# VCISwang/STCD

Measured on AMD Instinct MI355X. Metric: image-pairs/sec (256x256 bf16 SiamUnet_diff train), higher is better.
Workload: dtype bf16; 1 GPU; SiamUnet_diff(3,2) 256x256 full training step (fwd + cross_entropy + bwd + AdamW), 16 pairs/GPU, synthetic LEVIR-CD-shaped pairs resident in HBM; global_batch=16, image=256, parallelism=dp1

## Files before the change

### stcd_amd/csrc/common.h

```cpp
#pragma once
#include <hip/hip_runtime.h>
#include <stdint.h>
#include <stdio.h>
#include <stdlib.h>
#include <string>
#include <string.h>

#include "../../include/stcd_hip.h"

namespace stcd {

typedef __bf16 bf16;

enum DType { F32 = STCD_DTYPE_F32, BF16 = STCD_DTYPE_BF16 };
inline size_t dsize(int dt) { return dt == BF16 ? 2 : 4; }

void set_error(const std::string& msg);

static inline int env_int(const char* name, int dflt) { const char* v = getenv(name); return v ? atoi(v) : dflt; }
static inline bool env_flag(const char* name, bool dflt) { const char* v = getenv(name); return v && v[0] == (dflt ? '0' : '1') ? !dflt : dflt; }

#define STCD_CHECK(cond, msg)                                              \
    do {                                                                   \
        if (!(cond)) {                                                     \
// ... 157 lines not shown
}
__device__ __forceinline__ void xf_fold8(const float* __restrict__ tab_sc, const float* __restrict__ tab_sh, const float4 m0, const float4 m1,
                                         float (&sc)[8], float (&sh)[8]) {
    const float mk[8] = {m0.x, m0.y, m0.z, m0.w, m1.x, m1.y, m1.z, m1.w};
#pragma unroll
    for (int j = 0; j < 8; ++j) { sc[j] = tab_sc[j] * mk[j]; sh[j] = tab_sh[j] * mk[j]; }
}


void launch_in_pack(int dt, const float* x1, const float* x2, void* X, int B, int cin, int H, int W, hipStream_t s, int dates = 2);
void launch_gout_pack(int dt, const float* g, void* G, int B, int L, int H, int W, hipStream_t s, long long* bias_acc = nullptr);
struct BiasJob { int64_t acc_off; int64_t out_off; int C, valid; float scale; int pad_; };
void launch_bias_finish(const BiasJob* jobs_dev, int njobs, const char* ws, float* grads, hipStream_t s);

void launch_conv_ref(int dt, const stcd_conv_geom& g, const void* in, const float* w, int kpad, int wld,
                     const float* bias, void* out, bool out_nchw_f32, hipStream_t s);
void launch_wgrad_ref(int dt, const stcd_conv_geom& g, const void* in, const void* dout, float* dw, int kpad, int wld,
                      hipStream_t s);
void launch_wgrad_ref_f64(int dt, const stcd_conv_geom& g, const void* in, const void* dout, double* dw, int kpad, int wld,
                          hipStream_t s);

struct ConvMfmaPlan {
    int CiB = 0, nchunks = 0, KS = 0, modeB = 0, NT = 0, NTtot = 0;
    int64_t wf_elems = 0;
    bool ok = false;
};
ConvMfmaPlan conv_mfma_plan(const stcd_conv_geom& g);
void launch_pack_frag(const stcd_conv_geom& g, const ConvMfmaPlan& p, const float* w, int kpad, int wld, void* dst,
                      hipStream_t s);
int launch_conv_mfma(const stcd_conv_geom& g, const ConvMfmaPlan& p, const void* in, const void* wf, const float* bias,
                     void* out, bool out_nchw_f32, hipStream_t s);
int launch_conv_mfma_x4(const stcd_conv_geom g[4], const ConvMfmaPlan p[4], const void* in, const void* const wf[4],
                        const float* bias, void* out, hipStream_t s);
struct ConvResPlan {
    int NT = 0, CW = 32, nslices = 0, P = 0, blocks = 0;
    int filt_bytes = 0, lds_bytes = 0;
    int single_halo = 0;
    bool ok = false;
};
ConvResPlan conv_res_plan(const stcd_conv_geom& g, const ConvMfmaPlan& p, int groups);
struct BwdSum {
    const void* Y = nullptr; int ldy = 0;
    const float* stat = nullptr;
    const float* mask = nullptr;
    long long* acc = nullptr;
    int groups = 1;
};
int launch_conv_res(const stcd_conv_geom& g, const ConvMfmaPlan& p, const ConvResPlan& rp, const void* in, const void* wf,
                    const float* bias, void* out, int groups, long long* stat_acc, int cpad, hipStream_t s, int stat_c0 = 0,
                    float s1_scale = BN_FS1, float s2_scale = BN_FS2, const XfSrc* xf = nullptr, const BwdSum* bs = nullptr);
bool conv_res_bwdsum_ok(const stcd_conv_geom& g, const ConvResPlan& rp);
struct ConvTilePlan {
    int NT = 0, nparts = 0, nbuf = 0, nslices = 0, P = 0, blocks = 0, ntiles = 0;
    int filt_bytes = 0, lds_bytes = 0;
    bool ok = false;
};
ConvTilePlan conv_tile_plan(const stcd_conv_geom& g, const ConvMfmaPlan& p, int groups);
int launch_conv_tile(const stcd_conv_geom& g, const ConvMfmaPlan& p, const ConvTilePlan& tp, const void* in, const void* wf,
                     const float* bias, void* out, int groups, long long* stat_acc, int cpad, hipStream_t s, int stat_c0 = 0,
                     float s1_scale = BN_FS1, float s2_scale = BN_FS2);
struct ConvGemmPlan {
    int W = 0;
    int tiles_m = 0, tiles_n = 0, blocks = 0, lds_bytes = 0;
    int pix_chunks = 0;
    bool ok = false;
};
ConvGemmPlan conv_gemm_plan(const stcd_conv_geom& g, const ConvMfmaPlan& p, int groups);
struct ConvEpi {
    int relu = 0;
    const void* gate = nullptr; int ldg = 0;
    const void* res = nullptr; int ldr = 0;
    float alpha = 1.f, beta = 1.f;
};
int launch_conv_gemm(const stcd_conv_geom& g, const ConvMfmaPlan& p, const ConvGemmPlan& gp, const void* in, const void* wf,
                   const float* bias, void* out, int groups, long long* stat_acc, int cpad, hipStream_t s, int stat_c0 = 0,
                   float s1_scale = BN_FS1, float s2_scale = BN_FS2, const ConvEpi* epi = nullptr);
struct ConvHaloPlan {
    int NH = 0;
    int nslices = 0, P = 0, blocks = 0, lds_bytes = 0;
    bool ok = false;
};
ConvHaloPlan conv_halo_plan(const stcd_conv_geom& g, const ConvMfmaPlan& p);
int launch_conv_halo(const stcd_conv_geom& g, const ConvMfmaPlan& p, const ConvHaloPlan& hp, const void* in, const void* wf,
                     const float* bias, void* out, hipStream_t s, const ConvEpi* epi = nullptr);

struct ConvDmaPlan {
    int tiles_m = 0, tiles_n = 0, blocks = 0, lds_bytes = 0;
    bool ok = false;
};
ConvDmaPlan conv_dma_plan(const stcd_conv_geom& g, const ConvMfmaPlan& p);
int launch_conv_dma(const stcd_conv_geom& g, const ConvMfmaPlan& p, const ConvDmaPlan& dp, const void* in, const void* wf,
                    const float* bias, void* out, hipStream_t s, const ConvEpi* epi = nullptr);

bool conv_small_ok(const stcd_conv_geom& g, const ConvMfmaPlan& p);
int conv_small_blocks(const stcd_conv_geom& g, int groups);
int launch_conv_small(const stcd_conv_geom& g, const void* in, const void* wf_modeB, const float* bias, void* out,
                      bool out_nchw_f32, int groups, long long* stat_acc, int cpad, hipStream_t s, const XfSrc* xf = nullptr,
                      const BwdSum* bs = nullptr);
bool conv_small_bwdsum_ok(const stcd_conv_geom& g);
struct WgradMfmaPlan {
    int WCI = 1, NTW = 1, gx = 1, gy = 1, gz = 1;
    int64_t slab_floats = 0;
    int wi_valid = 0;
    int gemm = 0;
    int dma = 0;
    bool ok = false;
// ... 317 lines not shown
```

### stcd_amd/csrc/engine.hip

```cpp
#include <algorithm>
#include <climits>
#include <cstdint>
#include <array>
#include <cstring>
#include <memory>
#include <vector>

#include "common.h"

namespace stcd {

static thread_local std::string g_err;
void set_error(const std::string& msg) { g_err = msg; }

enum ConvKind { K_CONV3 = 0, K_CONVT3_S1 = 1, K_UPCONV = 2, K_CONV1 = 3, K_CONVT2 = 4, K_CONV3_S2 = 5, K_CONV1_S2 = 6, K_STEM7 = 7 };

struct TRef { int64_t off = -1; int ld = 0; };
struct GRef { int64_t off = -1; int ld = 0; int64_t goff = 0; };

static inline int round8(int c) { return (c + 7) & ~7; }

struct ConvW {
    std::string name;
    int kind = 0, cin = 0, cout = 0;
// ... 445 lines not shown
        if (e.convs[i].name == name) return (int)i;
    return -1;
}
static int bn_index(const stcd_engine& e, const std::string& name) {
    for (size_t i = 0; i < e.bns.size(); ++i)
        if (e.bns[i].name == name) return (int)i;
    return -1;
}

static stcd_conv_geom geom3(int N, int H, int W, int K, int ldi, int co, int ldo) {
    stcd_conv_geom g;
    memset(&g, 0, sizeof(g));
    g.n = N; g.hi = H; g.wi = W; g.ci = K; g.ldi = ldi;
    g.hm = H; g.wm = W; g.in_stride = 1;
    g.ho = H; g.wo = W; g.out_stride = 1; g.oy0 = 0; g.ox0 = 0;
    g.co = co; g.ldo = ldo;
    g.ntaps = 9;
    for (int t = 0; t < 9; ++t) { g.dy[t] = (int8_t)(t / 3 - 1); g.dx[t] = (int8_t)(t % 3 - 1); }
    return g;
}

static stcd_conv_geom geom_up_phase(const UpConv& U, int py, int px, int ldi, int ldo, int* tap0) {
    stcd_conv_geom g;
    memset(&g, 0, sizeof(g));
    g.n = U.N; g.hi = U.h; g.wi = U.w; g.ci = U.C; g.ldi = ldi;
    g.hm = U.h; g.wm = U.w; g.in_stride = 1;
    g.ho = U.Ho; g.wo = U.Wo; g.out_stride = 2; g.oy0 = py; g.ox0 = px;
    g.co = U.C; g.ldo = ldo;
    int t = 0;
    for (int dy = 0; dy <= py; ++dy)
        for (int dx = 0; dx <= px; ++dx) { g.dy[t] = (int8_t)dy; g.dx[t] = (int8_t)dx; ++t; }
    g.ntaps = t;
    static const int start[4] = {0, 1, 3, 5};
    *tap0 = start[py * 2 + px];
    return g;
}

static void conv_work(const stcd_engine& e, const stcd_conv_geom& g, int kreal, int nreal, double* flops, double* bytes);

static void pick_gemm_or_res(const stcd_engine& e, ConvOp& op, const stcd_conv_geom& g, int groups) {
    op.gemm = ConvGemmPlan();
    op.tile = ConvTilePlan();
    if (!e.use_gemm || op.small) return;
    if (op.res.ok && !(e.cf && op.res.NT == 1)) return;
    op.gemm = conv_gemm_plan(g, op.plan, groups);
    if (op.gemm.ok) op.res = ConvResPlan();
    static const bool halo_on = env_flag("STCD_HALO_KERNEL", false);
    op.halo = ConvHaloPlan();
    op.dma = ConvDmaPlan();
    if (op.gemm.ok && (int64_t)g.n * g.hm * g.wm >= 256 * 192) op.dma = conv_dma_plan(g, op.plan);
    if (halo_on && op.gemm.ok && (int64_t)g.n * ((g.hm + 15) / 16) * ((g.wm + 15) / 16) >= 512) op.halo = conv_halo_plan(g, op.plan);
}

constexpr int TILE_MAX_TILES = 512;
static void pick_tile(const stcd_engine& e, ConvOp& op, const stcd_conv_geom& g, int groups) {
    op.tile = ConvTilePlan();
    if (!e.use_tile || !op.res.ok || op.gemm.ok || op.small) return;
    const ConvTilePlan tp = conv_tile_plan(g, op.plan, groups);
    if (tp.ok && tp.ntiles <= TILE_MAX_TILES) op.tile = tp;
}

static WgradMfmaPlan pick_wgrad_plan(const stcd_engine& e, const stcd_conv_geom& g, int kpad, int wld) {
    if (e.use_gemm && e.use_wgroup && 2.0 * g.n * g.hm * g.wm * (double)g.ci * g.co >= 0.8e9) {
        WgradMfmaPlan p = wgrad_gemm_plan(g, kpad, wld);
        if (p.ok) return p;
    }
    if (e.use_wgroup && (g.ntaps == 9 || (e.cf && g.ntaps == 4)) && (int64_t)g.n * g.hm * g.wm >= 65536) {
        WgradMfmaPlan p = wgrad_dma_plan(g, kpad, wld);
        if (p.ok) return p;
    }
    return wgrad_mfma_plan(g, kpad, wld, is_snunet(e.arch) || (e.cf && g.ntaps == 9));
}

static bool same_group(const WgradGroup& G, const WgradOp& op) {
    const bool t9 = !op.plan.dma && op.g.ntaps == 9;
    return G.gemm == op.plan.gemm && G.dma == op.plan.dma && G.WCI == op.plan.WCI && G.NTW == op.plan.NTW && G.t9 == t9 && G.xf == (op.xf_C > 0);
}

static bool cf_side_on() { static const bool on = env_flag("STCD_CF_SIDE", true); return on; }

static void build_pack_jobs(stcd_engine& e, Bump& ws) {
    for (int st = 0; st < 2; ++st) { e.rjobs[st].clear(); e.rjobs_total[st] = 0; }
    for (int st = 0; st < 2; ++st) e.wgroups[st].clear();
    if (e.dt == BF16 && e.use_mfma) {
        if (e.use_wgroup) {
            for (WgradOp* op : e.wgrad_ops) {
                if (!op->plan.ok) continue;
                const bool t9 = !op->plan.dma && op->g.ntaps == 9;
                std::vector<WgradGroup>& gs = e.wgroups[op->stage];
                size_t gi = 0;
                while (gi < gs.size() && !same_group(gs[gi], *op)) ++gi;
                if (gi == gs.size()) { WgradGroup g; g.WCI = op->plan.WCI; g.NTW = op->plan.NTW; g.t9 = t9; g.gemm = op->plan.gemm; g.dma = op->plan.dma; g.xf = op->xf_C > 0; gs.push_back(g); }
                op->grouped = true;
            }
            for (int st = 0; st < 2; ++st)
                for (WgradGroup& G : e.wgroups[st]) {
                    if (G.gemm) { G.lds_bytes = 2 * 2 * G.gemm * (64 * 64 + 8 * 32); continue; }
                    if (G.dma) {
                        G.lds_bytes = 128 * 1024;
                        std::vector<WgradOp*> dops;
                        for (WgradOp* op : e.wgrad_ops)
                            if (op->grouped && op->stage == st && op->plan.dma) dops.push_back(op);
                        auto blocks_at = [&](int64_t kt) {
                            int64_t b = 0;
                            for (WgradOp* op : dops) {
                                const int64_t M = (int64_t)op->g.n * op->g.hi * op->g.wi;
                                b += ((M + kt * 64 - 1) / (kt * 64)) * op->plan.gy * op->plan.gz;
                            }
                            return b;
                        };
                        int64_t lo = 1, hi = 1;
                        const int dma_blocks = e.wg_side_on && cf_side_on() ? 192 : 256;
// ... 488 lines not shown
    hipStream_t s;
    template <typename P = void> P* at(int64_t off) const { return (P*)(ws + off); }
};

struct ProfScope {
    Prof& p; hipStream_t s; bool on; hipEvent_t b;
    ProfScope(const Ctx& c, int klass, double flops, double bytes, const char* kernel = nullptr);
    ~ProfScope() { if (on) (void)hipEventRecord(b, s); }
};

ProfScope::ProfScope(const Ctx& c, int klass, double flops, double bytes, const char* kernel)
    : p(c.e.prof), s(c.s), on(c.e.prof.on), b(nullptr) {
    if (!on) return;
    static const char* DEF[PC_COUNT] = {"k_conv", "k_wgrad", "k_bn_reduce<T, 0>", "k_bn_act", "k_bn_reduce<T, 1>", "k_bn_bwd_apply",
                                        "k_pool_bwd|k_fuse|k_slice", "k_pack_jobs|k_reduce_dw"};
    ProfRec r;
    r.a = p.get(); r.b = p.get(); r.klass = klass; r.flops = flops; r.bytes = bytes;
    r.name_id = p.intern(kernel ? kernel : DEF[klass]);
    b = r.b;
    p.recs.push_back(r);
    (void)hipEventRecord(r.a, s);
}

static void conv_work(const stcd_engine& e, const stcd_conv_geom& g, int kreal, int nreal, double* flops, double* bytes) {
    double pos = (double)g.n * g.hm * g.wm;
    *flops = 2.0 * pos * g.ntaps * kreal * nreal;
    double in_px = g.in_stride == 1 ? pos : (double)g.n * (2.0 * g.hm) * (2.0 * g.wm);
    *bytes = (in_px * kreal + pos * nreal + (double)g.ntaps * kreal * nreal) * (double)dsize(e.dt);
}

static bool mfma_on(const stcd_engine& e) { return e.dt == BF16 && e.use_mfma; }

struct StatReq { long long* acc = nullptr; int groups = 1; int c0 = 0; int C = 0; float s1 = BN_FS1, s2 = BN_FS2; };
static void exec_conv(const Ctx& c, const ConvOp& op, const void* in, const float* bias, void* out, bool nchw,
                      const StatReq* sr = nullptr, int* stat_chunks = nullptr, const ConvEpi* epi = nullptr, int* epi_fused = nullptr,
                      const XfSrc* xf = nullptr, const BwdSum* bs = nullptr) {
    const int stat_groups = (sr && sr->acc) ? sr->groups : 0;
    long long* stat_acc = sr ? sr->acc : nullptr;
    const bool bn_form = sr && sr->c0 == 0 && sr->C == op.g.co && sr->s1 == BN_FS1 && sr->s2 == BN_FS2;
    const ConvW& cv = c.e.convs[op.conv];
    const PackSpec& ps = op.dgrad ? cv.dgrad : cv.fwd;
    double fl, by;
    conv_work(c.e, op.g, op.kreal, op.nreal, &fl, &by);
    char kname[64];
    const bool gemm_path = mfma_on(c.e) && op.gemm.ok && op.wf >= 0 && !nchw;
    const bool small_path = !gemm_path && mfma_on(c.e) && op.small && op.wf >= 0 && c.e.use_small;
    const bool res_path = !gemm_path && !small_path && mfma_on(c.e) && op.res.ok && op.wf >= 0 && !nchw;
    const bool mfma_path = !small_path && !res_path && mfma_on(c.e) && op.plan.ok && op.wf >= 0;
    const bool tile_path = res_path && op.tile.ok && !(xf && xf->on) && !bs;
    const bool dma_path = gemm_path && op.dma.ok && op.res_groups == 1 && !(stat_groups > 0 && stat_acc);
    if (dma_path) snprintf(kname, sizeof(kname), "k_conv_dma");
    else if (gemm_path && op.halo.ok && !(stat_groups > 0 && stat_acc)) snprintf(kname, sizeof(kname), "k_conv_halo");
    else if (gemm_path) snprintf(kname, sizeof(kname), "k_conv_gemm<%d>", op.gemm.W);
    else if (tile_path) snprintf(kname, sizeof(kname), "k_conv_tile<%d>", op.tile.NT);
    else if (res_path) snprintf(kname, sizeof(kname), "k_conv_res<%d, %d, %s>", op.res.NT, op.res.CW, op.res.single_halo ? "true" : "false");
    else if (small_path) snprintf(kname, sizeof(kname), "k_conv_small<1, %d>", (op.g.ntaps * op.g.ci + 31) / 32 <= 5 ? 5 : 9);
    else if (mfma_path) snprintf(kname, sizeof(kname), "k_conv_mfma<%d>", op.plan.NT);
    else snprintf(kname, sizeof(kname), "k_conv_ref");
    if (bs) {
        ProfScope ps2(c, PC_CONV, fl, by + (double)op.g.n * op.g.ho * op.g.wo * op.g.co * 2.0, small_path ? "k_conv_small<bwd>" : "k_conv_res<bwd>");
        const int rc = small_path ? launch_conv_small(op.g, in, c.at(op.wf), bias, out, nchw, bs->groups, nullptr, op.g.co, c.s, nullptr, bs)
                                  : launch_conv_res(op.g, op.plan, op.res, in, c.at(op.wf), bias, out, op.res_groups, nullptr, op.g.co, c.s, 0,
                                                    BN_BS, BN_BS, nullptr, bs);
        if (rc != 0) set_error("fused BatchNorm-backward sums: the data-gradient launch does not fit its BWD kernel");
        return;
    }
    ProfScope prof(c, PC_CONV, fl, by, kname);
    if (stat_chunks) *stat_chunks = 0;
    if (epi_fused) *epi_fused = 0;
    if (dma_path && launch_conv_dma(op.g, op.plan, op.dma, in, c.at(op.wf), bias, out, c.s, epi) == 0) {
        if (epi_fused && epi) *epi_fused = 1;
        return;
    }
    if (gemm_path && op.halo.ok && !(stat_groups > 0 && stat_acc)) {
        if (launch_conv_halo(op.g, op.plan, op.halo, in, c.at(op.wf), bias, out, c.s, epi) == 0) {
            if (epi_fused && epi) *epi_fused = 1;
            return;
        }
    }
    if (gemm_path) {
        const bool want = stat_groups > 0 && stat_groups == op.res_groups && stat_acc;
        long long* sp = want ? stat_acc : nullptr;
        if (launch_conv_gemm(op.g, op.plan, op.gemm, in, c.at(op.wf), bias, out, op.res_groups, sp, want ? sr->C : op.g.co, c.s,
                           want ? sr->c0 : 0, want ? sr->s1 : BN_FS1, want ? sr->s2 : BN_FS2, epi) == 0) {
            if (stat_chunks && want) *stat_chunks = 1;
            if (epi_fused && epi) *epi_fused = 1;
            return;
        }
    }
    const bool xf_on = xf && xf->on;
    if (mfma_on(c.e) && op.small && op.wf >= 0 && c.e.use_small) {
        const int groups = xf_on ? xf->groups : (stat_groups > 0 && bn_form) ? stat_groups : 1;
        long long* sp = (stat_groups > 0 && bn_form && stat_groups == groups) ? stat_acc : nullptr;
        if (launch_conv_small(op.g, in, c.at(op.wf), bias, out, nchw, groups, sp, op.g.co, c.s, xf) == 0) {
            if (stat_chunks && sp) *stat_chunks = 1;
            return;
        }
    }
    if (tile_path) {
        const bool want = stat_groups > 0 && stat_groups == op.res_groups && stat_acc;
        long long* sp = want ? stat_acc : nullptr;
        if (launch_conv_tile(op.g, op.plan, op.tile, in, c.at(op.wf), bias, out, op.res_groups, sp, want ? sr->C : op.g.co, c.s,
                             want ? sr->c0 : 0, want ? sr->s1 : BN_FS1, want ? sr->s2 : BN_FS2) == 0) {
            if (stat_chunks && want) *stat_chunks = 1;
            return;
        }
    }
// ... 2242 lines not shown
    STCD_HIP(hipGetLastError());
    return 0;
}

static int check_geom(const stcd_conv_geom* g) {
    STCD_CHECK(g != nullptr, "geometry is null");
    STCD_CHECK(g->ntaps >= 1 && g->ntaps <= 9, "ntaps must be in [1,9]");
    STCD_CHECK(g->ci >= 8 && g->ci % 8 == 0 && g->ldi >= g->ci && g->ldi % 8 == 0, "ci/ldi must be multiples of 8");
    STCD_CHECK(g->co >= 1 && g->ldo >= g->co, "bad co/ldo");
    STCD_CHECK(g->in_stride >= 1 && g->out_stride >= 1 && g->n >= 1 && g->hm >= 1 && g->wm >= 1, "bad sizes");
    STCD_CHECK((g->hm - 1) * g->out_stride + g->oy0 < g->ho && (g->wm - 1) * g->out_stride + g->ox0 < g->wo,
               "output positions exceed the output buffer");
    return 0;
}
static int op_dma_splits(const stcd_conv_geom& g, const WgradMfmaPlan& p) {
    const int64_t M = (int64_t)g.n * g.hi * g.wi;
    return (int)std::max<int64_t>(1, std::min<int64_t>(256 / std::max(1, p.gy * p.gz), M / 512));
}
int64_t stcd_op_scratch_bytes(const stcd_conv_geom* g) {
    if (!g) return 0;
    ConvMfmaPlan p = conv_mfma_plan(*g);
    WgradMfmaPlan w = wgrad_mfma_plan(*g, g->ci, g->co), ww = wgrad_mfma_plan(*g, g->ci, g->co, true);
    WgradMfmaPlan wg = wgrad_gemm_plan(*g, g->ci, g->co);
    WgradMfmaPlan wd = wgrad_dma_plan(*g, g->ci, g->co);
    if (wd.ok) wgrad_dma_set_split(wd, *g, op_dma_splits(*g, wd), g->ci, g->co);
    return std::max<int64_t>(p.wf_elems * 2, std::max(std::max(std::max(w.slab_floats, ww.slab_floats), wg.ok ? wg.slab_floats : 0), wd.ok ? wd.slab_floats : 0) * 4) + 1024;
}
int stcd_op_conv(int dtype, int impl, const stcd_conv_geom* g, const void* in, const float* w, const float* bias,
                 void* out, void* scratch, int64_t scratch_bytes, void* hip_stream) {
    if (check_geom(g)) return 1;
    STCD_CHECK(in && w && out, "null pointer argument");
    if (impl == 1 || impl == 2 || impl == 3 || impl == 6 || impl == 8) {
        STCD_CHECK(dtype == STCD_DTYPE_BF16, "the MFMA implementation is bf16 only");
        ConvMfmaPlan p = conv_mfma_plan(*g);
        STCD_CHECK(p.ok, "geometry not supported by the MFMA kernel");
        STCD_CHECK(scratch && scratch_bytes >= p.wf_elems * 2, "scratch too small for the fragment-order filter");
        launch_pack_frag(*g, p, w, g->ci, g->co, scratch, (hipStream_t)hip_stream);
        if (impl == 3) {
            const ConvHaloPlan hp = conv_halo_plan(*g, p);
            STCD_CHECK(hp.ok, "geometry not supported by the resident-halo kernel (3x3 stride 1, Ci % 64 == 0, Co % 128 == 0)");
            STCD_CHECK(launch_conv_halo(*g, p, hp, in, scratch, bias, out, (hipStream_t)hip_stream) == 0, "launch failed");
            STCD_HIP(hipGetLastError());
            return 0;
        }
        if (impl == 6) {
            const ConvDmaPlan dp = conv_dma_plan(*g, p);
            STCD_CHECK(dp.ok, "geometry not supported by the LDS-DMA kernel (Ci % 64 == 0, Co % 256 == 0, (Ci / 64) * taps even and >= 4)");
            STCD_CHECK(launch_conv_dma(*g, p, dp, in, scratch, bias, out, (hipStream_t)hip_stream) == 0, "launch failed");
            STCD_HIP(hipGetLastError());
            return 0;
        }
        if (impl == 8) {
            const ConvTilePlan tp = conv_tile_plan(*g, p, 1);
            STCD_CHECK(tp.ok, "geometry not supported by the LDS-DMA tile kernel (3x3 stride 1 over the full map, Ci % 64 == 0, Co % 16 == 0)");
            STCD_CHECK(launch_conv_tile(*g, p, tp, in, scratch, bias, out, 1, nullptr, g->co, (hipStream_t)hip_stream) == 0, "launch failed");
            STCD_HIP(hipGetLastError());
            return 0;
        }
        if (impl == 1 && conv_small_ok(*g, p)) {
            STCD_CHECK(launch_conv_small(*g, in, scratch, bias, out, false, 1, nullptr, g->co, (hipStream_t)hip_stream) == 0,
                       "small-channel kernel rejected the geometry");
            STCD_HIP(hipGetLastError());
            return 0;
        }
        if (impl == 1 && !env_flag("STCD_NO_RES_KERNEL", false)) {
            const ConvResPlan rp = conv_res_plan(*g, p, 1);
            if (rp.ok && launch_conv_res(*g, p, rp, in, scratch, bias, out, 1, nullptr, g->co, (hipStream_t)hip_stream) == 0) {
                STCD_HIP(hipGetLastError());
                return 0;
            }
        }
        if (impl == 1 && !env_flag("STCD_NO_GEMM_KERNEL", false)) {
            const ConvGemmPlan gp = conv_gemm_plan(*g, p, 1);
            if (gp.ok && launch_conv_gemm(*g, p, gp, in, scratch, bias, out, 1, nullptr, g->co, (hipStream_t)hip_stream) == 0) {
                STCD_HIP(hipGetLastError());
                return 0;
            }
        }
        STCD_CHECK(launch_conv_mfma(*g, p, in, scratch, bias, out, false, (hipStream_t)hip_stream) == 0, "LDS budget exceeded");
        STCD_HIP(hipGetLastError());
        return 0;
    }
    STCD_CHECK(impl == 0, "impl must be 0 (reference FMA), 1 (MFMA, auto-selected kernel), 2 (generic MFMA kernel), 3 (resident-halo kernel), 6 (LDS-DMA kernel) or 8 (LDS-DMA tile kernel)");
    launch_conv_ref(dtype, *g, in, w, g->ci, g->co, bias, out, false, (hipStream_t)hip_stream);
    STCD_HIP(hipGetLastError());
    return 0;
}
int stcd_op_wgrad(int dtype, int impl, const stcd_conv_geom* g, const void* in, const void* dout, float* dw, void* scratch,
                  int64_t scratch_bytes, void* hip_stream) {
    if (check_geom(g)) return 1;
    STCD_CHECK(in && dout && dw, "null pointer argument");
    if (impl == 1 || impl == 4 || impl == 5) {
        STCD_CHECK(dtype == STCD_DTYPE_BF16, "the MFMA implementation is bf16 only");
        WgradMfmaPlan p = wgrad_mfma_plan(*g, g->ci, g->co, impl >= 4, impl == 5 ? 1 : 0);
        STCD_CHECK(p.ok, "geometry not supported by the MFMA kernel");
        STCD_CHECK(scratch && scratch_bytes >= p.slab_floats * 4, "scratch too small for the partial slabs");
        STCD_CHECK(launch_wgrad_mfma(*g, p, in, dout, (float*)scratch, g->ci, g->co, (hipStream_t)hip_stream) == 0, "LDS budget exceeded");
        launch_reduce_dw((const float*)scratch, p.gx, *g, g->ci, g->co, g->ci, g->co, nullptr, dw, (hipStream_t)hip_stream);
        STCD_HIP(hipGetLastError());
        return 0;
    }
    if (impl == 7) {
        STCD_CHECK(dtype == STCD_DTYPE_BF16, "the MFMA implementation is bf16 only");
        WgradMfmaPlan p = wgrad_dma_plan(*g, g->ci, g->co);
        STCD_CHECK(p.ok, "geometry not supported by the LDS-DMA weight-gradient kernel (stride 1, full map >= 64 wide, Ci % 256 == 0, Co % 256 == 0)");
        wgrad_dma_set_split(p, *g, op_dma_splits(*g, p), g->ci, g->co);
        const int64_t table = (p.slab_floats * 4 + 255) & ~(int64_t)255;
// ... 32 lines not shown
```

### stcd_amd/csrc/kernels_conv_tile.hip

```cpp
#include <algorithm>

#include "common.h"

namespace stcd {

typedef __attribute__((ext_vector_type(8))) __bf16 bf16x8;
typedef __attribute__((ext_vector_type(4))) float f32x4;
typedef __attribute__((ext_vector_type(2))) unsigned u32x2;

struct ConvTileArgs {
    stcd_conv_geom g;
    const bf16* in;
    const bf16* wf;
    const float* bias;
    bf16* out;
    int NTtot;
    int nparts, nbuf;
    int nslices, P, groups;
    int tiles_x, tiles_y, ntiles;
    int filt_bytes;
    long long* stat_acc;
    int cpad, stat_c0;
    float s1_scale, s2_scale;
    unsigned in_bytes, wf_bytes, out_bytes;
    int8_t tix[3][3];
};

constexpr int TL_HW = 18;
constexpr int TL_NDMA = 41;
constexpr int TL_PART = TL_NDMA * 1024;
constexpr int TL_NI = 11;
#define TL_LDS(P_) ((__attribute__((address_space(3))) void*)(P_))
#define TL_WAIT(N_) asm volatile("s_waitcnt vmcnt(%0)" ::"n"(N_) : "memory")

template <int NT>
__global__ void __launch_bounds__(256, NT == 4 ? 1 : 2)
k_conv_tile(const ConvTileArgs a) {
    extern __shared__ __attribute__((aligned(16))) char smem[];
    const int tid = threadIdx.x, lane = tid & 63;
    const int wid = __builtin_amdgcn_readfirstlane(tid >> 6);
    const int q = lane >> 4, r = lane & 15;
    const int P = a.P;
    const int bl = blockIdx.x % P, rest = blockIdx.x / P, slice = rest % a.nslices, grp = rest / a.nslices;
    char* const filt = smem;
    char* const halo0 = smem + a.filt_bytes;
    const int nparts = a.nparts, nbuf = a.nbuf;

    const int64_t lead = ((int64_t)a.g.wi + 1) * a.g.ldi * 2;
    const __amdgpu_buffer_rsrc_t xrs = __builtin_amdgcn_make_buffer_rsrc(
        const_cast<char*>(reinterpret_cast<const char*>(a.in)) - lead, (short)0, (int)(a.in_bytes + (unsigned)lead), 0x00020000);
    const __amdgpu_buffer_rsrc_t wrs = __builtin_amdgcn_make_buffer_rsrc(
        const_cast<char*>(reinterpret_cast<const char*>(a.wf)), (short)0, (int)a.wf_bytes, 0x00020000);
    const __amdgpu_buffer_rsrc_t ors = __builtin_amdgcn_make_buffer_rsrc(
        reinterpret_cast<char*>(a.out), (short)0, (int)a.out_bytes, 0x00020000);

    float bv[NT][4];
#pragma unroll
    for (int t2 = 0; t2 < NT; ++t2) {
        const int cb = (slice * NT + t2) * 16 + 4 * q;
        float4 b4 = make_float4(0.f, 0.f, 0.f, 0.f);
        if (a.bias) b4 = *reinterpret_cast<const float4*>(a.bias + cb);
        bv[t2][0] = b4.x; bv[t2][1] = b4.y; bv[t2][2] = b4.z; bv[t2][3] = b4.w;
    }
    asm volatile("s_waitcnt vmcnt(0)" ::: "memory");

    {
        const int nfrag = nparts * 2 * 9 * NT;
        for (int f0 = wid; f0 < nfrag + wid; f0 += 4) {
            const int f = min(f0, nfrag - 1);
            const int ntl = f % NT, ft = f / NT, t = ft % 9, c32 = ft / 9;
            const int src = (((c32 >> 1) * 9 + t) * 2 + (c32 & 1)) * a.NTtot + slice * NT + ntl;
            __builtin_amdgcn_raw_ptr_buffer_load_lds(wrs, TL_LDS(filt + f * 1024), 16, lane * 16,
                                                     __builtin_amdgcn_readfirstlane(src * 1024), 0, 0);
        }
    }

    int pyx[TL_NI], poff[TL_NI];
#pragma unroll
    for (int i = 0; i < TL_NI; ++i) {
        const int pix = min(wid + 4 * i, TL_NDMA - 1) * 8 + (lane >> 3);
        const int hx = pix % TL_HW, hy = pix / TL_HW;
        const int ch = (lane & 7) ^ ((hx >> 1) & 7);
        pyx[i] = pix < TL_HW * TL_HW ? (((hy - 1) << 16) | ((hx - 1) & 0xffff)) : (0x4000 << 16);
        poff[i] = ((hy * a.g.wi + hx) * a.g.ldi + ch * 8) * 2;
    }

    const int tpg = a.ntiles / a.groups;
// ... 115 lines not shown
                    acc[m][t2] = f32x4{0.f, 0.f, 0.f, 0.f};
                    u32x2 pk;
                    pk[0] = pack_bf16x2(v[0], v[1]);
                    pk[1] = pack_bf16x2(v[2], v[3]);
                    __builtin_amdgcn_raw_buffer_store_b64(pk, ors, inside ? (int)(obyte + t2 * 32) : (int)0x80000000u, 0, 0);
                    if (want_stats && inside) {
#pragma unroll
                        for (int j = 0; j < 4; ++j) {
                            const float rv = round_as<bf16>(v[j]);
                            s1[t2][j] += rv;
                            s2[t2][j] += rv * rv;
                        }
                    }
                }
            }
            stored = true;
        }
        TL_ADV(cur);
        buf = buf + 1 == nbuf ? 0 : buf + 1;
    }
#undef TL_ADV
#undef TL_REQ

    if (a.stat_acc) {
        float* red = reinterpret_cast<float*>(smem);
        __syncthreads();
#pragma unroll
        for (int t2 = 0; t2 < NT; ++t2)
#pragma unroll
            for (int j = 0; j < 4; ++j) {
                float x = s1[t2][j], y = s2[t2][j];
#pragma unroll
                for (int o = 1; o < 16; o <<= 1) { x += __shfl_xor(x, o, 64); y += __shfl_xor(y, o, 64); }
                if (r == 0) {
                    red[(((wid * NT + t2) * 4 + q) * 4 + j) * 2] = x;
                    red[(((wid * NT + t2) * 4 + q) * 4 + j) * 2 + 1] = y;
                }
            }
        __syncthreads();
        for (int i = tid; i < NT * 16 * 2; i += 256) {
            const int which = i / (NT * 16), c = i - which * NT * 16;
            const int t2 = c >> 4, qq = (c >> 2) & 3, j = c & 3;
            float acc_ = 0.f;
#pragma unroll
            for (int w = 0; w < 4; ++w) acc_ += red[(((w * NT + t2) * 4 + qq) * 4 + j) * 2 + which];
            const int chn = slice * NT * 16 + c - a.stat_c0;
            if (chn >= 0 && chn < a.cpad) bn_acc_add(a.stat_acc, bl, a.groups, a.cpad, grp, which, chn, acc_, which ? a.s2_scale : a.s1_scale);
        }
    }
}

ConvTilePlan conv_tile_plan(const stcd_conv_geom& g, const ConvMfmaPlan& p, int groups) {
    ConvTilePlan tp;
    if (!p.ok || p.modeB || p.CiB != 64 || g.ntaps != 9 || g.in_stride != 1 || g.out_stride != 1 || g.oy0 != 0 || g.ox0 != 0) return tp;
    if (g.ci % 64 != 0 || g.co % 16 != 0 || g.ldi % 8 != 0 || g.ldo % 4 != 0 || g.hm > g.hi || g.wm > g.wi) return tp;
    if (g.hm > g.ho || g.wm > g.wo) return tp;
    if (g.hi >= 16384 || g.wi >= 16384) return tp;
    if (groups < 1 || g.n % groups != 0) return tp;
    if (((int64_t)g.n * g.hi + 2) * g.wi * g.ldi * 2 >= ((int64_t)1 << 31)) return tp;
    if ((int64_t)g.n * g.ho * g.wo * g.ldo * 2 >= ((int64_t)1 << 31)) return tp;
    if ((int64_t)p.wf_elems * 2 >= ((int64_t)1 << 31)) return tp;
    bool seen[9] = {false};
    for (int t = 0; t < 9; ++t) {
        if (g.dy[t] < -1 || g.dy[t] > 1 || g.dx[t] < -1 || g.dx[t] > 1) return tp;
        seen[(g.dy[t] + 1) * 3 + g.dx[t] + 1] = true;
    }
    for (int t = 0; t < 9; ++t) if (!seen[t]) return tp;
    const int nparts = g.ci / 64, nbuf = std::min(nparts, 2), ntr = g.co / 16, cap = 160 * 1024 - 1024;
    auto lds_of = [&](int nt) { return nparts * 2 * 9 * nt * 1024 + nbuf * TL_PART; };
    int NT = 0;
    for (int nt = 4; nt >= 1 && !NT; nt >>= 1)
        if (ntr % nt == 0 && lds_of(nt) <= cap) NT = nt;
    if (!NT) return tp;
    if (NT == 4 && 2 * lds_of(2) <= cap) NT = 2;
    const int64_t tiles_x = (g.wm + 15) / 16, tiles_y = (g.hm + 15) / 16, ntiles = (int64_t)g.n * tiles_x * tiles_y;
    if (ntiles >= ((int64_t)1 << 24)) return tp;
    while (NT > 1 && ntiles * (ntr / NT) < 256) NT >>= 1;
    tp.NT = NT; tp.nparts = nparts; tp.nbuf = nbuf; tp.nslices = ntr / NT;
    tp.filt_bytes = nparts * 2 * 9 * NT * 1024;
    tp.lds_bytes = lds_of(NT);
    tp.ntiles = (int)ntiles;
    const int64_t tpg = ntiles / groups;
    const int per_cu = std::max(1, std::min(2, cap / tp.lds_bytes));
    const int64_t slots = (int64_t)per_cu * 256;
    const int64_t P = std::max<int64_t>(1, slots / ((int64_t)groups * tp.nslices));
    tp.P = (int)std::min<int64_t>(P, tpg);
    tp.blocks = tp.P * tp.nslices * groups;
    tp.ok = true;
    return tp;
}

int launch_conv_tile(const stcd_conv_geom& g, const ConvMfmaPlan& p, const ConvTilePlan& tp, const void* in, const void* wf,
                     const float* bias, void* out, int groups, long long* stat_acc, int cpad, hipStream_t s, int stat_c0, float s1_scale,
                     float s2_scale) {
    if (!tp.ok || groups < 1 || tp.blocks != tp.P * tp.nslices * groups) return 1;
    ConvTileArgs a;
    a.g = g;
    a.in = (const bf16*)in; a.wf = (const bf16*)wf; a.bias = bias; a.out = (bf16*)out;
    a.NTtot = p.NTtot; a.nparts = tp.nparts; a.nbuf = tp.nbuf;
    a.nslices = tp.nslices; a.P = tp.P; a.groups = groups;
    a.tiles_x = (g.wm + 15) / 16; a.tiles_y = (g.hm + 15) / 16; a.ntiles = g.n * a.tiles_x * a.tiles_y;
    a.filt_bytes = tp.filt_bytes;
    a.stat_acc = stat_acc; a.cpad = cpad; a.stat_c0 = stat_c0; a.s1_scale = s1_scale; a.s2_scale = s2_scale;
    a.in_bytes = (unsigned)((int64_t)g.n * g.hi * g.wi * g.ldi * 2);
    a.wf_bytes = (unsigned)(p.wf_elems * 2);
    a.out_bytes = (unsigned)((int64_t)g.n * g.ho * g.wo * g.ldo * 2);
    for (int t = 0; t < 9; ++t) a.tix[g.dy[t] + 1][g.dx[t] + 1] = (int8_t)t;
#define LAUNCH_TILE(N_)                                                                                           \
    do {                                                                                                          \
        static bool attr_set = false;                                                                             \
        if (!attr_set) {                                                                                          \
            (void)hipFuncSetAttribute((const void*)k_conv_tile<N_>, hipFuncAttributeMaxDynamicSharedMemorySize, 160 * 1024); \
            attr_set = true;                                                                                      \
        }                                                                                                         \
        k_conv_tile<N_><<<(unsigned)tp.blocks, 256, (size_t)tp.lds_bytes, s>>>(a);                                \
    } while (0)
    switch (tp.NT) {
        case 1: LAUNCH_TILE(1); break;
        case 2: LAUNCH_TILE(2); break;
        default: LAUNCH_TILE(4); break;
    }
#undef LAUNCH_TILE
    return 0;
}

}
```

Before: 7915 image-pairs/sec.

## Extend LDS-DMA tile conv kernel to 32-channel input parts and raise tile cap

Adds a templated tile-conv body that handles 32-channel input parts (CiB==32) with its own swizzle, multi-buffer halo ring (up to four buffers), and vmcnt-based waiting, so more 3x3 convs can take the LDS-DMA tile path instead of the res kernel. It also raises the maximum tile count eligible for the tile path from 512 to 1024, gated by a check that the stats partition matches the res plan. The goal is better overlap of halo loads with MFMA work on small-channel layers. Risks include lower arithmetic intensity per part and changed BN stat accumulation ordering.

```diff
diff --git a/stcd_amd/csrc/common.h b/stcd_amd/csrc/common.h
--- a/stcd_amd/csrc/common.h
+++ b/stcd_amd/csrc/common.h
@@ -233,6 +233,7 @@
 bool conv_res_bwdsum_ok(const stcd_conv_geom& g, const ConvResPlan& rp);
 struct ConvTilePlan {
     int NT = 0, nparts = 0, nbuf = 0, nslices = 0, P = 0, blocks = 0, ntiles = 0;
+    int PC = 64;
     int filt_bytes = 0, lds_bytes = 0;
     bool ok = false;
 };
diff --git a/stcd_amd/csrc/engine.hip b/stcd_amd/csrc/engine.hip
--- a/stcd_amd/csrc/engine.hip
+++ b/stcd_amd/csrc/engine.hip
@@ -521,12 +521,19 @@
     if (halo_on && op.gemm.ok && (int64_t)g.n * ((g.hm + 15) / 16) * ((g.wm + 15) / 16) >= 512) op.halo = conv_halo_plan(g, op.plan);
 }
 
-constexpr int TILE_MAX_TILES = 512;
+struct TilePick { int PC, max_tiles; };
+static const TilePick TILE_PICKS[] = {
+    {64, 1024},
+    {32, 1024},
+};
 static void pick_tile(const stcd_engine& e, ConvOp& op, const stcd_conv_geom& g, int groups) {
     op.tile = ConvTilePlan();
     if (!e.use_tile || !op.res.ok || op.gemm.ok || op.small) return;
     const ConvTilePlan tp = conv_tile_plan(g, op.plan, groups);
-    if (tp.ok && tp.ntiles <= TILE_MAX_TILES) op.tile = tp;
+    if (!tp.ok) return;
+    const bool same_sums = op.dgrad || tp.P == op.res.P || (tp.PC == 64 && tp.ntiles <= 512);
+    for (const TilePick& r : TILE_PICKS)
+        if (tp.PC == r.PC && tp.ntiles <= r.max_tiles && same_sums) { op.tile = tp; return; }
 }
 
 static WgradMfmaPlan pick_wgrad_plan(const stcd_engine& e, const stcd_conv_geom& g, int kpad, int wld) {
@@ -1121,7 +1128,7 @@
     if (dma_path) snprintf(kname, sizeof(kname), "k_conv_dma");
     else if (gemm_path && op.halo.ok && !(stat_groups > 0 && stat_acc)) snprintf(kname, sizeof(kname), "k_conv_halo");
     else if (gemm_path) snprintf(kname, sizeof(kname), "k_conv_gemm<%d>", op.gemm.W);
-    else if (tile_path) snprintf(kname, sizeof(kname), "k_conv_tile<%d>", op.tile.NT);
+    else if (tile_path) snprintf(kname, sizeof(kname), op.tile.PC == 64 ? "k_conv_tile<%d>" : "k_conv_tile_parts<%d, 32>", op.tile.NT);
     else if (res_path) snprintf(kname, sizeof(kname), "k_conv_res<%d, %d, %s>", op.res.NT, op.res.CW, op.res.single_halo ? "true" : "false");
     else if (small_path) snprintf(kname, sizeof(kname), "k_conv_small<1, %d>", (op.g.ntaps * op.g.ci + 31) / 32 <= 5 ? 5 : 9);
     else if (mfma_path) snprintf(kname, sizeof(kname), "k_conv_mfma<%d>", op.plan.NT);
@@ -3470,7 +3477,7 @@
         }
         if (impl == 8) {
             const ConvTilePlan tp = conv_tile_plan(*g, p, 1);
-            STCD_CHECK(tp.ok, "geometry not supported by the LDS-DMA tile kernel (3x3 stride 1 over the full map, Ci % 64 == 0, Co % 16 == 0)");
+            STCD_CHECK(tp.ok, "geometry not supported by the LDS-DMA tile kernel (3x3 stride 1 over the full map, Ci % 32 == 0, Co % 16 == 0)");
             STCD_CHECK(launch_conv_tile(*g, p, tp, in, scratch, bias, out, 1, nullptr, g->co, (hipStream_t)hip_stream) == 0, "launch failed");
             STCD_HIP(hipGetLastError());
             return 0;
diff --git a/stcd_amd/csrc/kernels_conv_tile.hip b/stcd_amd/csrc/kernels_conv_tile.hip
--- a/stcd_amd/csrc/kernels_conv_tile.hip
+++ b/stcd_amd/csrc/kernels_conv_tile.hip
@@ -27,12 +27,309 @@
 };
 
 constexpr int TL_HW = 18;
+constexpr int TL_MAXBUF = 4;
+template <int PC> struct TilePart {
+    static constexpr int NCH = PC / 8;
+    static constexpr int PPI = 64 / NCH;
+    static constexpr int NDMA = (TL_HW * TL_HW + PPI - 1) / PPI;
+    static constexpr int BYTES = NDMA * 1024;
+    static constexpr int NI = (NDMA + 3) / 4;
+    static constexpr int KS = PC / 32;
+};
+#define TL_LDS(P_) ((__attribute__((address_space(3))) void*)(P_))
+#define TL_WAIT(N_) asm volatile("s_waitcnt vmcnt(%0)" ::"n"(N_) : "memory")
+
+constexpr int TL_SWZ[TL_HW] = {3, 0, 1, 2, 7, 7, 5, 2, 3, 4, 4, 5, 7, 7, 0, 1, 3, 0};
+constexpr uint64_t tl_swz_pack() {
+    uint64_t v = 0;
+    for (int c = 0; c < TL_HW; ++c) v |= (uint64_t)TL_SWZ[c] << (3 * c);
+    return v;
+}
+constexpr uint64_t TL_SWZ_BITS = tl_swz_pack();
+template <int PC> __host__ __device__ constexpr int tl_swz(int col) {
+    return PC == 64 ? (int)((TL_SWZ_BITS >> (3 * col)) & 7) : (col >> 1) & 3;
+}
+template <int PC> constexpr bool tl_swz_conflict_free() {
+    constexpr int NCH = TilePart<PC>::NCH;
+    constexpr int g0[16] = {0, 1, 2, 3, 12, 13, 14, 15, 20, 21, 22, 23, 24, 25, 26, 27};
+    for (int c = 0; c < TL_HW; ++c)
+        if (tl_swz<PC>(c) < 0 || tl_swz<PC>(c) >= NCH) return false;
+    for (int row = 0; row < TL_HW; ++row)
+        for (int ks = 0; ks < TilePart<PC>::KS; ++ks)
+            for (int dx = 0; dx < 3; ++dx)
+                for (int grp = 0; grp < 4; ++grp) {
+                    unsigned seen = 0;
+                    for (int l = 0; l < 32; ++l) {
+                        bool in0 = false;
+                        for (int i = 0; i < 16; ++i) in0 = in0 || g0[i] == l;
+                        if (in0 != ((grp & 1) == 0)) continue;
+                        const int lane = l + 32 * (grp >> 1), q = lane >> 4, r = lane & 15;
+                        const int byte = ((row * TL_HW + r + dx) * NCH + ((ks * 4 + q) ^ tl_swz<PC>(r + dx))) * 16;
+                        const unsigned bit = 1u << ((byte >> 4) & 15);
+                        if (seen & bit) return false;
+                        seen |= bit;
+                    }
+                    if (seen != 0xffffu) return false;
+                }
+    return true;
+}
+static_assert(tl_swz_conflict_free<64>(), "a shifted halo fragment read has an LDS bank conflict (128-B pixel rows)");
+static_assert(tl_swz_conflict_free<32>(), "a shifted halo fragment read has an LDS bank conflict (64-B pixel rows)");
+
+__device__ __forceinline__ void tl_wait_vm(int n) {
+    switch (n) {
+#define TL_W1(N_) case N_: TL_WAIT(N_); break;
+#define TL_W8(N_) TL_W1(N_) TL_W1(N_ + 1) TL_W1(N_ + 2) TL_W1(N_ + 3) TL_W1(N_ + 4) TL_W1(N_ + 5) TL_W1(N_ + 6) TL_W1(N_ + 7)
+        TL_W8(0) TL_W8(8) TL_W8(16) TL_W8(24) TL_W8(32) TL_W8(40) TL_W8(48) TL_W8(56)
+#undef TL_W8
+#undef TL_W1
+        default: TL_WAIT(0); break;
+    }
+}
+
+template <int NT, int PC>
+__device__ __forceinline__ void conv_tile_body(const ConvTileArgs& a) {
+    using TP = TilePart<PC>;
+    constexpr int TL_NDMA = TP::NDMA, TL_PART = TP::BYTES, TL_NI = TP::NI, TL_KS = TP::KS, TL_NCH = TP::NCH, TL_PPI = TP::PPI;
+    extern __shared__ __attribute__((aligned(16))) char smem[];
+    const int tid = threadIdx.x, lane = tid & 63;
+    const int wid = __builtin_amdgcn_readfirstlane(tid >> 6);
+    const int q = lane >> 4, r = lane & 15;
+    const int P = a.P;
+    const int bl = blockIdx.x % P, rest = blockIdx.x / P, slice = rest % a.nslices, grp = rest / a.nslices;
+    char* const filt = smem;
+    char* const halo0 = smem + a.filt_bytes;
+    const int nparts = a.nparts, nbuf = a.nbuf;
+
+    const int64_t lead = ((int64_t)a.g.wi + 1) * a.g.ldi * 2;
+    const __amdgpu_buffer_rsrc_t xrs = __builtin_amdgcn_make_buffer_rsrc(
+        const_cast<char*>(reinterpret_cast<const char*>(a.in)) - lead, (short)0, (int)(a.in_bytes + (unsigned)lead), 0x00020000);
+    const __amdgpu_buffer_rsrc_t wrs = __builtin_amdgcn_make_buffer_rsrc(
+        const_cast<char*>(reinterpret_cast<const char*>(a.wf)), (short)0, (int)a.wf_bytes, 0x00020000);
+    const __amdgpu_buffer_rsrc_t ors = __builtin_amdgcn_make_buffer_rsrc(
+        reinterpret_cast<char*>(a.out), (short)0, (int)a.out_bytes, 0x00020000);
+
+    float bv[NT][4];
+#pragma unroll
+    for (int t2 = 0; t2 < NT; ++t2) {
+        const int cb = (slice * NT + t2) * 16 + 4 * q;
+        float4 b4 = make_float4(0.f, 0.f, 0.f, 0.f);
+        if (a.bias) b4 = *reinterpret_cast<const float4*>(a.bias + cb);
+        bv[t2][0] = b4.x; bv[t2][1] = b4.y; bv[t2][2] = b4.z; bv[t2][3] = b4.w;
+    }
+    asm volatile("s_waitcnt vmcnt(0)" ::: "memory");
+#pragma unroll
+    for (int t2 = 0; t2 < NT; ++t2)
+#pragma unroll
+        for (int j = 0; j < 4; ++j) asm volatile("" : "+v"(bv[t2][j]));
+
+    constexpr int TL_PF = TL_KS * 9 * NT, TL_NF = (TL_PF + 3) / 4;
+#define TL_REQ_FILT(C_)                                                                                                \
+    do {                                                                                                               \
+        _Pragma("unroll") for (int i = 0; i < TL_NF; ++i) {                                                            \
+            const int f = (C_) * TL_PF + min(wid + 4 * i, TL_PF - 1);                                                  \
+            const int ntl = f % NT, ft = f / NT, t = ft % 9, c32 = ft / 9;                                             \
+            const int src = (((c32 / TL_KS) * 9 + t) * TL_KS + c32 % TL_KS) * a.NTtot + slice * NT + ntl;              \
+            __builtin_amdgcn_raw_ptr_buffer_load_lds(wrs, TL_LDS(filt + f * 1024), 16, lane * 16,                      \
+                                                     __builtin_amdgcn_readfirstlane(src * 1024), 0, 0);                \
+        }                                                                                                              \
+    } while (0)
+
+    int pyx[TL_NI], poff[TL_NI];
+#pragma unroll
+    for (int i = 0; i < TL_NI; ++i) {
+        const int pix = min(wid + 4 * i, TL_NDMA - 1) * TL_PPI + lane / TL_NCH;
+        const int hx = pix % TL_HW, hy = pix / TL_HW;
+        const int ch = (lane % TL_NCH) ^ tl_swz<PC>(hx);
+        pyx[i] = pix < TL_HW * TL_HW ? (((hy - 1) << 16) | ((hx - 1) & 0xffff)) : (0x4000 << 16);
+        poff[i] = ((hy * a.g.wi + hx) * a.g.ldi + ch * 8) * 2;
+    }
+
+    const int tpg = a.ntiles / a.groups;
+    const int tiles_img = a.tiles_x * a.tiles_y;
+    const int dn = P / tiles_img, drem = P - dn * tiles_img, dty = drem / a.tiles_x, dtx = drem - dty * a.tiles_x;
+    const int tile0 = grp * tpg + bl;
+    const int tile_end = (grp + 1) * tpg;
+    struct Pos { int tile, n, y, x, c; };
+#define TL_ADV(P_)                                                                                                     \
+    do {                                                                                                               \
+        if (++(P_).c == nparts) {                                                                                      \
+            (P_).c = 0; (P_).tile += P;                                                                                \
+            (P_).x += dtx; if ((P_).x >= a.tiles_x) { (P_).x -= a.tiles_x; ++(P_).y; }                                 \
+            (P_).y += dty; if ((P_).y >= a.tiles_y) { (P_).y -= a.tiles_y; ++(P_).n; }                                 \
+            (P_).n += dn;                                                                                              \
+        }                                                                                                              \
+    } while (0)
+#define TL_REQ(P_, BUF_)                                                                                               \
+    do {                                                                                                               \
+        const int gy0_ = (P_).y * 16, gx0_ = (P_).x * 16;                                                               \
+        const int soff_ = __builtin_amdgcn_readfirstlane(                                                              \
+            (int)(((((int64_t)(P_).n * a.g.hi + gy0_) * a.g.wi + gx0_) * a.g.ldi + (P_).c * PC) * 2));                 \
+        char* const dst_ = halo0 + (BUF_) * TL_PART;                                                                   \
+        _Pragma("unroll") for (int i = 0; i < TL_NI; ++i) {                                                            \
+            const int hy_ = pyx[i] >> 16, hx_ = (int)(short)(pyx[i] & 0xffff);                                         \
+            const bool ok_ = (unsigned)(gy0_ + hy_) < (unsigned)a.g.hi && (unsigned)(gx0_ + hx_) < (unsigned)a.g.wi;   \
+            __builtin_amdgcn_raw_ptr_buffer_load_lds(xrs, TL_LDS(dst_ + min(wid + 4 * i, TL_NDMA - 1) * 1024), 16,     \
+                                                     ok_ ? poff[i] : (int)0x80000000u, soff_, 0, 0);                   \
+        }                                                                                                              \
+    } while (0)
+
+    Pos cur{tile0, 0, 0, 0, 0};
+    cur.n = tile0 / tiles_img;
+    { const int trem = tile0 - cur.n * tiles_img; cur.y = trem / a.tiles_x; cur.x = trem - cur.y * a.tiles_x; }
+    Pos rq = cur;
+    int inflight = 0;
+    for (int k = 0; k < nbuf; ++k) {
+        if (k < nparts) TL_REQ_FILT(k);
+        if (rq.tile < tile_end) { TL_REQ(rq, k); TL_ADV(rq); ++inflight; }
+    }
+    for (int k = nbuf; k < nparts; ++k) TL_REQ_FILT(k);
+#undef TL_REQ_FILT
+
+    float s1[NT][4], s2[NT][4];
+#pragma unroll
+    for (int t2 = 0; t2 < NT; ++t2)
+#pragma unroll
+        for (int j = 0; j < 4; ++j) s1[t2][j] = s2[t2][j] = 0.f;
+    f32x4 acc[4][NT];
+#pragma unroll
+    for (int m = 0; m < 4; ++m)
+#pragma unroll
+        for (int t2 = 0; t2 < NT; ++t2) acc[m][t2] = f32x4{0.f, 0.f, 0.f, 0.f};
+
+    int aoff[TL_KS][3];
+#pragma unroll
+    for (int ks = 0; ks < TL_KS; ++ks)
+#pragma unroll
+        for (int dx = 0; dx < 3; ++dx)
+            aoff[ks][dx] = (((4 * wid) * TL_HW + r + dx) * TL_NCH + ((ks * 4 + q) ^ tl_swz<PC>(r + dx))) * 16;
+
+    const bool want_stats = a.stat_acc != nullptr;
+    int buf = 0, step = 0;
+    unsigned ended = 0;
+    const unsigned ring = (1u << nbuf) - 1;
+    while (cur.tile < tile_end) {
+        {
+            const int ny = inflight - 1;
+            const int nst = __builtin_popcount(ended & ring);
+            tl_wait_vm(ny * TL_NI + nst * 4 * NT + (step < nbuf ? max(nparts - 1 - step, 0) * TL_NF : 0));
+            --inflight;
+        }
+        __builtin_amdgcn_s_barrier();
+        const char* hb = halo0 + buf * TL_PART;
+        {
+            bf16x8 ab[2][6], wb[2][3][NT];
+            const char* const fb0 = filt + (cur.c * TL_KS) * (9 * NT * 1024) + lane * 16;
+#define TL_LOAD_STAGE(S_, B_)                                                                                         \
+            do {                                                                                                      \
+                constexpr int ks_ = (S_) / 3, dx_ = (S_) % 3;                                                         \
+                _Pragma("unroll") for (int hr = 0; hr < 6; ++hr)                                                      \
+                    ab[B_][hr] = *reinterpret_cast<const bf16x8*>(hb + aoff[ks_][dx_] + hr * (TL_HW * PC * 2));       \
+                _Pragma("unroll") for (int dy = 0; dy < 3; ++dy)                                                      \
+                    _Pragma("unroll") for (int t2 = 0; t2 < NT; ++t2)                                                 \
+                        wb[B_][dy][t2] = *reinterpret_cast<const bf16x8*>(fb0 + ks_ * (9 * NT * 1024) + a.tix[dy][dx_] * (NT * 1024) + t2 * 1024); \
+            } while (0)
+#define TL_MMA_STAGE(B_)                                                                                              \
+            do {                                                                                                      \
+                _Pragma("unroll") for (int dy = 0; dy < 3; ++dy)                                                      \
+                    _Pragma("unroll") for (int t2 = 0; t2 < NT; ++t2)                                                 \
+                        _Pragma("unroll") for (int m = 0; m < 4; ++m)                                                 \
+                            acc[m][t2] = __builtin_amdgcn_mfma_f32_16x16x32_bf16(wb[B_][dy][t2], ab[B_][m + dy], acc[m][t2], 0, 0, 0); \
+            } while (0)
+            TL_LOAD_STAGE(0, 0);
+            TL_LOAD_STAGE(1, 1); __builtin_amdgcn_sched_barrier(0);
+            TL_MMA_STAGE(0);
+            TL_LOAD_STAGE(2, 0); __builtin_amdgcn_sched_barrier(0);
+            TL_MMA_STAGE(1);
+            if constexpr (TL_KS == 2) {
+                TL_LOAD_STAGE(3, 1); __builtin_amdgcn_sched_barrier(0);
+                TL_MMA_STAGE(0);
+                TL_LOAD_STAGE(4, 0); __builtin_amdgcn_sched_barrier(0);
+                TL_MMA_STAGE(1);
+                TL_LOAD_STAGE(5, 1); __builtin_amdgcn_sched_barrier(0);
+                TL_MMA_STAGE(0);
+                TL_MMA_STAGE(1);
+            } else {
+                TL_MMA_STAGE(0);
+            }
+#undef TL_LOAD_STAGE
+#undef TL_MMA_STAGE
+        }
+        barrier_lds();
+        if (rq.tile < tile_end) { TL_REQ(rq, buf); TL_ADV(rq); ++inflight; }
+        if (cur.c == nparts - 1) {
+            const int mx = cur.x * 16 + r;
+#pragma unroll
+            for (int m = 0; m < 4; ++m) {
+                const int my = cur.y * 16 + wid * 4 + m;
+                const bool inside = my < a.g.hm && mx < a.g.wm;
+                const unsigned obyte = (unsigned)(((((int64_t)cur.n * a.g.ho + my) * a.g.wo + mx) * a.g.ldo + slice * NT * 16 + 4 * q) * 2);
+#pragma unroll
+                for (int t2 = 0; t2 < NT; ++t2) {
+                    float v[4];
+#pragma unroll
+                    for (int j = 0; j < 4; ++j) v[j] = acc[m][t2][j] + bv[t2][j];
+                    acc[m][t2] = f32x4{0.f, 0.f, 0.f, 0.f};
+                    u32x2 pk;
+                    pk[0] = pack_bf16x2(v[0], v[1]);
+                    pk[1] = pack_bf16x2(v[2], v[3]);
+                    __builtin_amdgcn_raw_buffer_store_b64(pk, ors, inside ? (int)(obyte + t2 * 32) : (int)0x80000000u, 0, 0);
+                    if (want_stats && inside) {
+#pragma unroll
+                        for (int j = 0; j < 4; ++j) {
+                            const float rv = round_as<bf16>(v[j]);
+                            s1[t2][j] += rv;
+                            s2[t2][j] += rv * rv;
+                        }
+                    }
+                }
+            }
+        }
+        ended = (ended << 1) | (cur.c == nparts - 1 ? 1u : 0u);
+        TL_ADV(cur);
+        buf = buf + 1 == nbuf ? 0 : buf + 1;
+        ++step;
+    }
+#undef TL_ADV
+#undef TL_REQ
+
+    if (a.stat_acc) {
+        float* red = reinterpret_cast<float*>(smem);
+        __syncthreads();
+#pragma unroll
+        for (int t2 = 0; t2 < NT; ++t2)
+#pragma unroll
+            for (int j = 0; j < 4; ++j) {
+                float x = s1[t2][j], y = s2[t2][j];
+#pragma unroll
+                for (int o = 1; o < 16; o <<= 1) { x += __shfl_xor(x, o, 64); y += __shfl_xor(y, o, 64); }
+                if (r == 0) {
+                    red[(((wid * NT + t2) * 4 + q) * 4 + j) * 2] = x;
+                    red[(((wid * NT + t2) * 4 + q) * 4 + j) * 2 + 1] = y;
+                }
+            }
+        __syncthreads();
+        for (int i = tid; i < NT * 16 * 2; i += 256) {
+            const int which = i / (NT * 16), c = i - which * NT * 16;
+            const int t2 = c >> 4, qq = (c >> 2) & 3, j = c & 3;
+            float acc_ = 0.f;
+#pragma unroll
+            for (int w = 0; w < 4; ++w) acc_ += red[(((w * NT + t2) * 4 + qq) * 4 + j) * 2 + which];
+            const int chn = slice * NT * 16 + c - a.stat_c0;
+            if (chn >= 0 && chn < a.cpad) bn_acc_add(a.stat_acc, bl, a.groups, a.cpad, grp, which, chn, acc_, which ? a.s2_scale : a.s1_scale);
+        }
+    }
+}
+
+template <int NT, int PC>
+__global__ void __launch_bounds__(256, 2)
+k_conv_tile_parts(const ConvTileArgs a) {
+    conv_tile_body<NT, PC>(a);
+}
+
 constexpr int TL_NDMA = 41;
 constexpr int TL_PART = TL_NDMA * 1024;
 constexpr int TL_NI = 11;
-#define TL_LDS(P_) ((__attribute__((address_space(3))) void*)(P_))
-#define TL_WAIT(N_) asm volatile("s_waitcnt vmcnt(%0)" ::"n"(N_) : "memory")
-
 template <int NT>
 __global__ void __launch_bounds__(256, NT == 4 ? 1 : 2)
 k_conv_tile(const ConvTileArgs a) {
@@ -254,8 +551,8 @@
 
 ConvTilePlan conv_tile_plan(const stcd_conv_geom& g, const ConvMfmaPlan& p, int groups) {
     ConvTilePlan tp;
-    if (!p.ok || p.modeB || p.CiB != 64 || g.ntaps != 9 || g.in_stride != 1 || g.out_stride != 1 || g.oy0 != 0 || g.ox0 != 0) return tp;
-    if (g.ci % 64 != 0 || g.co % 16 != 0 || g.ldi % 8 != 0 || g.ldo % 4 != 0 || g.hm > g.hi || g.wm > g.wi) return tp;
+    if (!p.ok || p.modeB || (p.CiB != 64 && p.CiB != 32) || g.ntaps != 9 || g.in_stride != 1 || g.out_stride != 1 || g.oy0 != 0 || g.ox0 != 0) return tp;
+    if (g.ci % p.CiB != 0 || g.co % 16 != 0 || g.ldi % 8 != 0 || g.ldo % 4 != 0 || g.hm > g.hi || g.wm > g.wi) return tp;
     if (g.hm > g.ho || g.wm > g.wo) return tp;
     if (g.hi >= 16384 || g.wi >= 16384) return tp;
     if (groups < 1 || g.n % groups != 0) return tp;
@@ -268,19 +565,34 @@
         seen[(g.dy[t] + 1) * 3 + g.dx[t] + 1] = true;
     }
     for (int t = 0; t < 9; ++t) if (!seen[t]) return tp;
-    const int nparts = g.ci / 64, nbuf = std::min(nparts, 2), ntr = g.co / 16, cap = 160 * 1024 - 1024;
-    auto lds_of = [&](int nt) { return nparts * 2 * 9 * nt * 1024 + nbuf * TL_PART; };
-    int NT = 0;
-    for (int nt = 4; nt >= 1 && !NT; nt >>= 1)
-        if (ntr % nt == 0 && lds_of(nt) <= cap) NT = nt;
-    if (!NT) return tp;
-    if (NT == 4 && 2 * lds_of(2) <= cap) NT = 2;
     const int64_t tiles_x = (g.wm + 15) / 16, tiles_y = (g.hm + 15) / 16, ntiles = (int64_t)g.n * tiles_x * tiles_y;
     if (ntiles >= ((int64_t)1 << 24)) return tp;
+    const int PC = p.CiB, nparts = g.ci / PC, ntr = g.co / 16, cap = 160 * 1024 - 1024;
+    const int part = PC == 64 ? TL_PART : TilePart<32>::BYTES, ni = TilePart<32>::NI;
+    auto filt_of = [&](int nt) { return nparts * (PC / 32) * 9 * nt * 1024; };
+    int NT = 0, nbuf = 0;
+    if (PC == 64) {
+        nbuf = std::min(nparts, 2);
+        auto lds_of = [&](int nt) { return filt_of(nt) + nbuf * part; };
+        for (int nt = 4; nt >= 1 && !NT; nt >>= 1)
+            if (ntr % nt == 0 && lds_of(nt) <= cap) NT = nt;
+        if (!NT) return tp;
+        if (NT == 4 && 2 * lds_of(2) <= cap) NT = 2;
+    } else {
+        for (int nt = 2; nt >= 1 && !NT; nt >>= 1)
+            if (ntr % nt == 0 && filt_of(nt) + part <= cap) NT = nt;
+        if (!NT) return tp;
+    }
     while (NT > 1 && ntiles * (ntr / NT) < 256) NT >>= 1;
-    tp.NT = NT; tp.nparts = nparts; tp.nbuf = nbuf; tp.nslices = ntr / NT;
-    tp.filt_bytes = nparts * 2 * 9 * NT * 1024;
-    tp.lds_bytes = lds_of(NT);
+    if (PC == 32) {
+        const int nf = ((PC / 32) * 9 * NT + 3) / 4;
+        nbuf = std::min(TL_MAXBUF, (cap / 2 - filt_of(NT)) / part);
+        if (nbuf < 2) nbuf = std::max(1, std::min(TL_MAXBUF, (cap - filt_of(NT)) / part));
+        while (nbuf > 1 && (nbuf - 1) * ni + nbuf * 4 * NT + (nparts - 1) * nf > 63) --nbuf;
+    }
+    tp.NT = NT; tp.PC = PC; tp.nparts = nparts; tp.nbuf = nbuf; tp.nslices = ntr / NT;
+    tp.filt_bytes = filt_of(NT);
+    tp.lds_bytes = tp.filt_bytes + nbuf * part;
     tp.ntiles = (int)ntiles;
     const int64_t tpg = ntiles / groups;
     const int per_cu = std::max(1, std::min(2, cap / tp.lds_bytes));
@@ -295,7 +607,8 @@
 int launch_conv_tile(const stcd_conv_geom& g, const ConvMfmaPlan& p, const ConvTilePlan& tp, const void* in, const void* wf,
                      const float* bias, void* out, int groups, long long* stat_acc, int cpad, hipStream_t s, int stat_c0, float s1_scale,
                      float s2_scale) {
-    if (!tp.ok || groups < 1 || tp.blocks != tp.P * tp.nslices * groups) return 1;
+    if (!tp.ok || groups < 1 || tp.blocks != tp.P * tp.nslices * groups || tp.PC != p.CiB || (tp.NT == 4 && tp.PC != 64)) return 1;
+    if (tp.nbuf < 1 || tp.nbuf > TL_MAXBUF) return 1;
     ConvTileArgs a;
     a.g = g;
     a.in = (const bf16*)in; a.wf = (const bf16*)wf; a.bias = bias; a.out = (bf16*)out;
@@ -308,19 +621,19 @@
     a.wf_bytes = (unsigned)(p.wf_elems * 2);
     a.out_bytes = (unsigned)((int64_t)g.n * g.ho * g.wo * g.ldo * 2);
     for (int t = 0; t < 9; ++t) a.tix[g.dy[t] + 1][g.dx[t] + 1] = (int8_t)t;
-#define LAUNCH_TILE(N_)                                                                                           \
+#define LAUNCH_TILE(K_)                                                                                            \
     do {                                                                                                          \
         static bool attr_set = false;                                                                             \
         if (!attr_set) {                                                                                          \
-            (void)hipFuncSetAttribute((const void*)k_conv_tile<N_>, hipFuncAttributeMaxDynamicSharedMemorySize, 160 * 1024); \
+            (void)hipFuncSetAttribute((const void*)K_, hipFuncAttributeMaxDynamicSharedMemorySize, 160 * 1024);                  \
             attr_set = true;                                                                                      \
         }                                                                                                         \
-        k_conv_tile<N_><<<(unsigned)tp.blocks, 256, (size_t)tp.lds_bytes, s>>>(a);                                \
+        K_<<<(unsigned)tp.blocks, 256, (size_t)tp.lds_bytes, s>>>(a);                                             \
     } while (0)
     switch (tp.NT) {
-        case 1: LAUNCH_TILE(1); break;
-        case 2: LAUNCH_TILE(2); break;
-        default: LAUNCH_TILE(4); break;
+        case 1: if (tp.PC == 64) LAUNCH_TILE(k_conv_tile<1>); else LAUNCH_TILE((k_conv_tile_parts<1, 32>)); break;
+        case 2: if (tp.PC == 64) LAUNCH_TILE(k_conv_tile<2>); else LAUNCH_TILE((k_conv_tile_parts<2, 32>)); break;
+        default: LAUNCH_TILE(k_conv_tile<4>); break;
     }
 #undef LAUNCH_TILE
     return 0;
```

Measured after the change: 7857 image-pairs/sec. About the same (-0.7%).
